# soytony/Point-Cloud-Preprocessing-Tools

Measured on AMD Instinct MI355X. Metric: BEV frames/sec (131k-pt HDL-64E cloud), higher is better.
Workload: dtype f32; 1 GPU; 1000 synthetic hdl64_sweep HDL_64E clouds per GPU (mean 135646 input pts, 133312 slots), single+multi BEV, device-resident; frames_per_gpu=1000, sub_batch=500, sensor=HDL_64E, parallelism=frames x1

## Files before the change

### point-cloud-preprocessing-tools_amd/csrc/bev_capi.hip

```cpp
#include <algorithm>
#include <cmath>
#include <cstdio>
#include <cstdlib>
#include <cstring>
#include <new>

#include <roctracer/roctx.h>

#include "bev_ctx.h"
#include "bev_libm.h"

using namespace bevk;
using namespace bevh;

namespace bevh {
void Downloader::run()
{
    (void)hipSetDevice(c->device);
    const size_t S = (size_t)c->geo.S;
    for (;;) {
        Task t;
        {
            std::unique_lock<std::mutex> lk(mu);
            cv.wait(lk, [&] { return closing || !queue.empty(); });
// ... 255 lines not shown
        HIPCK(c, hipEventRecord(c->null_ev, nullptr));
        if (!fused) HIPCK(c, hipStreamWaitEvent(c->stream, c->null_ev, 0));
        for (int q = 0; fused && q < c->n_stage_streams; ++q) HIPCK(c, hipStreamWaitEvent(c->stage_st[q], c->null_ev, 0));
    }

    int ds = 0;
    if (!identity) {
        int rc = acquire_desc(c, (size_t)n_frames, &ds);
        if (rc != BEV_OK) return rc;
        for (int f = 0; f < n_frames; ++f) {
            const uint64_t a = h_offsets[f], b = h_offsets[f + 1];
            if (b < a || b - a > c->max_points) {
                c->desc_used[ds] = false;
                return BEV_ERR_TOO_LARGE;
            }
            c->h_desc[ds][f].in_offset = a;
            c->h_desc[ds][f].n_pts = (uint32_t)(b - a);
            c->h_desc[ds][f]._pad = 0;
        }
    }

    const int sub_size = sub_frames > 0 ? std::min(sub_frames, c->max_batch) : c->max_batch;
    for (int f0 = 0; f0 < n_frames; f0 += sub_size) {
        const int nb = std::min(sub_size, n_frames - f0);
        const int q = fused ? (int)(c->sub_seq % (unsigned)c->n_stage_streams) : 0;
        hipStream_t st = fused ? c->stage_st[q] : c->stream;
        Lane &ln = c->lanes[c->sub_seq % (unsigned)c->n_lanes];
        ++c->sub_seq;
        BatchPtrs b{};
        b.pts = identity ? d_pts + (size_t)f0 * S : d_pts;
        b.frames = identity ? nullptr : ln.desc;
        b.frames_src = identity ? nullptr : c->d_desc[ds] + f0;
        b.frames_copy = identity ? nullptr : ln.desc;
        b.info = identity ? nullptr : ln.info;
        b.est = ln.est;
        b.tail_list = ln.tail_list;
        b.tail_cnt = ln.tail_cnt;
        b.cm_par = ln.cm_par;
        b.cm_sync = ln.cm_sync;
        b.winner = ln.winner;
        b.win_shift = c->win_shift;
        b.ordered = d_ordered + (size_t)f0 * S;
        b.cand = ln.cand;
        b.ncand = ln.ncand;
        b.code_main = ln.code_main;
        b.ncode = ln.ncode;
        b.ctx_tab = c->ctx_tab;
        b.avg = ln.avg;
        b.gm = d_gm ? ln.gm : nullptr;
        b.multi = d_multi ? d_multi + (size_t)f0 * c->multi_bytes : nullptr;
        b.single = d_single ? d_single + (size_t)f0 * c->single_bytes : nullptr;

        bool carried = !fused;
        auto walk = [&](int kid, int source, uint32_t mode) -> int {
            if (!carried) {
                carried = true;
                StageArgs a{};
                a.g = g;
                a.walk.b = b;
                a.walk.nf = nb;
                a.want_mode = mode;
                a.lead = c->stage_lead;
                if (!pending_is_consistent(c, q)) {
                    const int rc_ = flush_pending(c);
                    if (rc_ != BEV_OK) return rc_;
                }
                take_pending(c, &a, q);
                if (source == kSrcColMajor || source == kSrcColMajorGen) {
                    {
                        ProfScope ps(c, kid, nb, st);
                        launch_gather_ground(g, b, nb, source, mode, st);
                    }
                    a.walk.nf = 0;
                    a.lead = 0;
                    ProfScope ps(c, K_STAGE, 0, st);
                    launch_stage(a, -1, st);
                } else {
                    ProfScope ps(c, K_STAGE, nb, st);
                    launch_stage(a, source, st);
                }
                return advance_pending(c, q);
            }
            ProfScope ps(c, kid, nb, st);
            launch_gather_ground(g, b, nb, source, mode, st);
            return BEV_OK;
        };

        if (identity) {
            RoctxRange rr("bev:front (identity walk)");
            int rc = walk(K_GATHER_GROUND, kSrcIdentity, kFrameGeneral);
            if (rc != BEV_OK) return rc;
        } else {
            RoctxRange rr("bev:front (probe, column walk beside the later stages of earlier sub-batches, verdict, order scan)");
            uint32_t max_pts = 0;
            int n_exact_s = 0;
            for (int f = 0; f < nb; ++f) {
                max_pts = std::max(max_pts, c->h_desc[ds][f0 + f].n_pts);
                n_exact_s += c->h_desc[ds][f0 + f].n_pts == (uint32_t)g.S ? 1 : 0;
            }
            const uint32_t max_gen = c->win_shift <= 28 ? (1u << (32 - c->win_shift)) - 1u : 0u;
            if (ln.win_gen + 1u > max_gen) {
                HIPCK(c, hipMemsetAsync(ln.winner, 0, (size_t)c->max_batch * S * sizeof(uint32_t), st));
                ln.win_gen = 0;
            }
            if (max_gen) ++ln.win_gen;
            b.win_tag = ln.win_gen;
            {
                ProfScope ps(c, K_PROBE, nb, st);
                launch_probe(g, b, nb, c->allow_stream, c->layout_hint, st);
            }
            uint32_t seen = 0u;
            if (c->allow_stream && c->hint) {
                const uint32_t word = reinterpret_cast<volatile uint32_t *>(c->hint)[1];
                for (int m = 0; m < 8; ++m) {
                    c->mode_absent[m] = (word >> m) & 1u ? 0 : std::min(c->mode_absent[m] + 1, 1 << 20);
                    if (c->mode_absent[m] < c->mode_ttl) seen |= 1u << m;
                }
            }
            if (c->layout_hint) seen |= 1u << c->layout_hint;
            int rc = BEV_OK;
            if (c->allow_stream && ln.tail_list && (seen & (1u << kFrameStream)))
                rc = walk(K_GATHER_GROUND, kSrcInPlace, kFrameStream);
            if (rc == BEV_OK && c->allow_stream && n_exact_s > 0 && (seen & (1u << kFrameStructured)))
                rc = walk(K_WALK_STRUCTURED, kSrcStructured, kFrameStructured);
            if (rc == BEV_OK && c->allow_stream && n_exact_s > 0 && (seen & (1u << kFrameColMajor)))
                rc = walk(K_WALK_COLMAJOR, kSrcColMajor, kFrameColMajor);
            if (rc == BEV_OK && c->allow_stream && n_exact_s > 0 && ln.cm_par && (seen & (1u << kFrameColMajorGen)))
                rc = walk(K_WALK_COLMAJOR_GEN, kSrcColMajorGen, kFrameColMajorGen);
            if (rc != BEV_OK) return rc;
            if (c->allow_stream) {
                ProfScope ps(c, K_VERDICT, nb, st);
                launch_verdict(g, b, nb, c->hint, st);
            }
            {
                const bool thin = c->allow_stream && c->hint && *reinterpret_cast<volatile uint32_t *>(c->hint) == 0u;
                ProfScope ps(c, K_ORDER_SCAN, nb, st);
                launch_order_scan(g, b, nb, max_pts, thin, st);
            }
            rc = walk(K_WALK_GENERAL, kSrcGather, kFrameGeneral);
            if (rc != BEV_OK) return rc;
        }
        if (fused) {
            c->pending.push_back(bev_ctx::Pending{b, nb, d_multi != nullptr, d_single != nullptr, d_gm ? d_gm + (size_t)f0 * S : nullptr, 1, q});
        } else {
            RoctxRange rb("bev:back (cell sums, resolve, rasters)");
            {
                ProfScope ps(c, K_CELL_SUMS, nb, st);
                launch_cell_sums(g, b, nb, st);
            }
            if (d_gm) {
                ProfScope ps(c, K_GROUND_MAT, nb, st);
                launch_ground_mat(g, b, d_gm + (size_t)f0 * S, nb, st);
            }
            {
                ProfScope ps(c, K_GROUND_RESOLVE, nb, st);
                launch_ground_resolve(g, b, nb, st);
            }
            if (d_multi || d_single) {
                ProfScope ps(c, K_BEV_RASTER, nb, st);
                launch_bev_raster(g, b, d_multi != nullptr, d_single != nullptr, nb, st);
            }
        }
        c->last_sub_frames = nb;
        c->last_avg = ln.avg;
        c->last_ncode = ln.ncode;
        c->last_info = identity ? nullptr : ln.info;
        HIPCK(c, hipGetLastError());
    }
    if (fused) {
        int rc = flush ? flush_pending(c) : join_stage_streams(c);
        if (rc != BEV_OK) return rc;
    }
    if (!identity) {
        HIPCK(c, hipEventRecord(c->desc_done[ds], c->stream));
        c->desc_used[ds] = true;
    }
    return BEV_OK;
}
}

namespace {

int process_batch_host(bev_ctx_t *c, int kind, int n_frames, const void *const *in, const uint32_t *n_pts,
                       bev_point_t *const *ordered_out, uint8_t *const *multi_out, uint8_t *const *single_out,
                       int8_t *const *ground_mat_out)
{
    if (!c || n_frames < 0 || (n_frames > 0 && (!in || !n_pts || !ordered_out))) return BEV_ERR_INVALID_ARG;
    const bool raw = kind >= 0, kitti = kind == BEV_PROJECT_KITTI_HDL_64E;
    const size_t in_size = raw ? 16 : sizeof(bev_point_t);
    if (kitti && (size_t)c->geo.S > c->max_points) return BEV_ERR_TOO_LARGE;
    for (int f = 0; f < n_frames; ++f) {
        if (n_pts[f] > (kitti ? std::max(c->max_points, (size_t)c->geo.S) : c->max_points)) return BEV_ERR_TOO_LARGE;
// ... 722 lines not shown
```

### point-cloud-preprocessing-tools_amd/csrc/bev_front.h

```cpp
#ifndef BEV_FRONT_H
#define BEV_FRONT_H

#include "bev_dev.h"

namespace bevk {
using namespace bevx;

#ifndef BEV_PROBE_THREADS
#define BEV_PROBE_THREADS 256
#endif
constexpr int kProbeThreads = BEV_PROBE_THREADS;
struct ProbeLds {
    uint32_t samp[kMaxSamples];
    union {
        struct {
            uint16_t col[kCmMaxSamples], col1[kCmMaxSamples];
            uint32_t ref[kCmMaxRows], lo[kCmMaxRows], hi[kCmMaxRows], base[kCmMaxRows], misc[4];
        } cm;
        uint32_t tcnt[kTailBuckets];
    } u;
    uint32_t first_bad, overflow, struct_bad, struct_zero, cm_bad, cm_not_plain;
};
static_assert(sizeof(ProbeLds) <= kSlotLdsBytes, "a quarter of a CU's LDS");
__device__ __forceinline__ void probe_body(char *arena, const BatchPtrs &b, const Geometry &g, int allow_stream, int layout_hint, const int f)
// ... 251 lines not shown
    __syncthreads();
    uint32_t *flist = b.tail_list + (size_t)f * g.N * g.strips * kTailCap;
    auto append = [&](int row, int strip, int off, uint32_t i) {
        const int bucket = row * g.strips + strip;
        const uint32_t pos = atomicAdd(&tcnt[bucket], 1u);
        if (pos < (uint32_t)kTailCap) flist[(size_t)bucket * kTailCap + pos] = (uint32_t)off | (i << 8);
        else overflow = 1u;
    };
    constexpr int kPer = 20;
    for (uint32_t i0 = T; i0 < n; i0 += (uint32_t)kProbeThreads * kPer) {
        uint32_t rc[kPer];
#pragma unroll
        for (int k = 0; k < kPer; ++k) {
            const uint32_t i = i0 + (uint32_t)kProbeThreads * k + tid;
            rc[k] = load_once(reinterpret_cast<const uint32_t *>(fp + (i < n ? i : n - 1u)) + 5);
        }
#pragma unroll
        for (int k = 0; k < kPer; ++k) {
            const uint32_t i = i0 + (uint32_t)kProbeThreads * k + tid;
            const int row = (int)(rc[k] & 0xffffu), col = (int)(rc[k] >> 16);
            if (i >= n || row >= g.N || col >= g.H) continue;
            const int st = col / kStripCols, c = col - st * kStripCols;
            append(row, st, c + 2, i);
            if (c < 2 && st > 0) append(row, st - 1, kStripCols + 2 + c, i);
            if (c >= kStripCols - 2 && st + 1 < g.strips) append(row, st + 1, c - (kStripCols - 2), i);
            if (col >= g.H - 2 && row + 1 < g.N) append(row + 1, 0, col - (g.H - 2), i);
            if (col < 2) {
                for (int ws = g.strips - 1; ws >= 0 && ws >= g.strips - 2; --ws) {
                    const int off = g.H + col - (ws * kStripCols - 2);
                    if (off < kStripVirt && ws * kStripCols < g.H) append(row, ws, off, i);
                }
            }
        }
    }
    __syncthreads();
    PH();
    uint32_t *fcnt = b.tail_cnt + (size_t)f * g.N * g.strips;
    for (int i = tid; i < g.N * g.strips; i += kProbeThreads) {
        const int r = i / g.strips, st = i - r * g.strips;
        fcnt[st * g.N + r] = tcnt[i] < (uint32_t)kTailCap ? tcnt[i] : (uint32_t)kTailCap;
    }
    if (tid == 0) b.info[f] = overflow ? FrameInfo{0u, kFrameGeneral, 4u, 0u} : FrameInfo{T, kFrameStream, 0u, 0u};
    PH();
    TL_END(K_PROBE);
    PH_PRINT("probe samples prefix-end estimates tail-lists counts", tid == 0 && f == 100);
}
__global__ __launch_bounds__(kProbeThreads) void k_probe(BatchPtrs b, Geometry g, int allow_stream, int layout_hint)
{
    __shared__ __attribute__((aligned(16))) char arena[sizeof(ProbeLds)];
    probe_body(arena, b, g, allow_stream, layout_hint, (int)blockIdx.x);
}


__global__ __launch_bounds__(1024) void k_verdict(FrameInfo *info, int nf, uint32_t *host_hint, const uint32_t *cm_sync, int N)
{
    __shared__ uint32_t others, modes;
    if (threadIdx.x == 0) others = modes = 0u;
    __syncthreads();
    uint32_t mine = 0u, mask = 0u;
    for (int f = threadIdx.x; f < nf; f += 1024) {
        FrameInfo fi = info[f];
        mask |= 1u << (fi.mode & 31u);
        bool bad_stream = ((fi.mode == kFrameStream || fi.mode == kFrameColMajor) && (fi.failed != 0u || fi.consumed != fi.T)) ||
                          (fi.mode == kFrameColMajorGen && ((fi.failed & kInfoFailed) != 0u || fi.consumed != fi.T));
        if (fi.mode == kFrameColMajorGen && !bad_stream && (fi.failed & (kInfoCmUsed | kInfoCmStray)) != 0u && cm_sync) {
            const uint32_t *win0 = cm_sync + (size_t)f * kCmSyncWords + kCmPubWords, *used0 = win0 + kCmMaxRows, *stray = used0 + kCmMaxRows;
            for (int r = 0; r < N && r < kCmMaxRows; ++r) {
                const uint32_t u = used0[r];
                if ((u & kCmUsedBit) != 0u && (u & ~kCmUsedBit) != win0[r]) bad_stream = true;
                if (stray[r] > win0[r]) bad_stream = true;
            }
        }
        const bool bad_struct = fi.mode == kFrameStructured &&
                                ((fi.failed & kInfoFailed) != 0u || fi.consumed != fi.T ||
                                 ((fi.failed & kInfoZeroSeen) != 0u) != ((fi.failed & kInfoZeroGuess) != 0u));
        if (bad_stream || bad_struct) {
            info[f].mode = kFrameRedo;
            fi.mode = kFrameRedo;
        }
        mine += frame_read_in_place(fi.mode) ? 0u : 1u;
    }
    if (mine) atomicAdd(&others, mine);
    if (mask) atomicOr(&modes, mask);
    __syncthreads();
    if (threadIdx.x == 0 && host_hint) {
        __hip_atomic_store(host_hint, others, __ATOMIC_RELAXED, __HIP_MEMORY_SCOPE_SYSTEM);
        __hip_atomic_store(host_hint + 1, modes, __ATOMIC_RELAXED, __HIP_MEMORY_SCOPE_SYSTEM);
    }
}

constexpr int kSeenBits = 11;
constexpr int kScanPerThread = 4;
constexpr int kScanIdxBits = 10;
constexpr int kScanRowBins = 128;
__global__ __launch_bounds__(256) void k_order_scan(const bev_point_t *__restrict__ pts,
                                                    const FrameDesc *__restrict__ frames,
                                                    const FrameInfo *__restrict__ info,
                                                    uint32_t *__restrict__ winner, int N, int H, int S,
                                                    uint32_t tag_bits)
{
    const int f = blockIdx.y;
    if (info && frame_read_in_place(info[f].mode)) return;
    const FrameDesc fd = frames[f];
    const bev_point_t *fp = pts + fd.in_offset;
    uint32_t *fw = winner + (size_t)f * S;
    __shared__ uint32_t any_spread2[2];
    __shared__ uint32_t row_fill[kScanRowBins];
    __shared__ uint32_t pairs[256 * kScanPerThread];
    static_assert(256 * kScanPerThread == (1 << kScanIdxBits), "bits of block-local index");
  uint32_t turn = 0u;
  for (uint32_t blk = blockIdx.x; blk * (256u * kScanPerThread) < fd.n_pts; blk += gridDim.x, ++turn) {
    uint32_t &any_spread = any_spread2[turn & 1u];
    const uint32_t block0 = blk * (256u * kScanPerThread);
    const uint32_t base = block0 + threadIdx.x;
    uint32_t slot[kScanPerThread];
    bool spread = false;
    uint32_t rcw[kScanPerThread];
#pragma unroll
    for (int k = 0; k < kScanPerThread; ++k) {
        const uint32_t i = base + 256u * k;
        rcw[k] = load_once(reinterpret_cast<const uint32_t *>(fp + (i < fd.n_pts ? i : fd.n_pts - 1u)) + 5);
    }
#pragma unroll
    for (int k = 0; k < kScanPerThread; ++k) {
        const uint32_t i = base + 256u * k;
        const uint32_t row = rcw[k] & 0xffffu, col = rcw[k] >> 16;
        slot[k] = (i < fd.n_pts && row < (uint32_t)N && col < (uint32_t)H) ? row * (uint32_t)H + col
                                                                                         : 0xffffffffu;
    }
#pragma unroll
    for (int k = 0; k < kScanPerThread; ++k) {
        const unsigned long long vm = __ballot(slot[k] != 0xffffffffu);
        if (vm) {
            const int lo_lane = __ffsll((long long)vm) - 1, hi_lane = 63 - __clzll((long long)vm);
            const uint32_t a = __shfl(slot[k], lo_lane), z = __shfl(slot[k], hi_lane);
            const uint32_t d = a > z ? a - z : z - a;
            spread = spread || d > 4u * (uint32_t)H;
        }
    }
    if (threadIdx.x == 0) any_spread = 0u;
    __syncthreads();
    if (spread && (threadIdx.x & 63) == 0) any_spread = 1u;
    __syncthreads();
    if (any_spread == 0u || N > kScanRowBins || S > (1 << (32 - kScanIdxBits))) {
#pragma unroll
        for (int k = 0; k < kScanPerThread; ++k)
            if (slot[k] != 0xffffffffu) atomicMax(&fw[slot[k]], tag_bits | (base + 256u * k + 1u));
        continue;
    }
    for (int r = threadIdx.x; r < kScanRowBins; r += 256) row_fill[r] = 0u;
#pragma unroll
    for (int k = 0; k < kScanPerThread; ++k) pairs[threadIdx.x + 256u * k] = 0xffffffffu;
    __syncthreads();
    uint32_t rank[kScanPerThread];
#pragma unroll
    for (int k = 0; k < kScanPerThread; ++k)
        rank[k] = slot[k] != 0xffffffffu ? atomicAdd(&row_fill[slot[k] / (uint32_t)H], 1u) : 0u;
    __syncthreads();
    if (threadIdx.x < 64) {
        const uint32_t c0 = row_fill[2 * threadIdx.x], c1 = row_fill[2 * threadIdx.x + 1];
        uint32_t incl = c0 + c1;
#pragma unroll
        for (int d = 1; d < 64; d <<= 1) {
            const uint32_t v = __shfl_up(incl, d);
            if ((int)threadIdx.x >= d) incl += v;
        }
        row_fill[2 * threadIdx.x] = incl - c0 - c1;
        row_fill[2 * threadIdx.x + 1] = incl - c1;
    }
    __syncthreads();
#pragma unroll
    for (int k = 0; k < kScanPerThread; ++k)
        if (slot[k] != 0xffffffffu)
            pairs[row_fill[slot[k] / (uint32_t)H] + rank[k]] = (slot[k] << kScanIdxBits) | (threadIdx.x + 256u * k);
    __syncthreads();
#pragma unroll
    for (int k = 0; k < kScanPerThread; ++k) {
        const uint32_t j = threadIdx.x + 256u * k;
        const uint32_t pr = pairs[j];
        if (pr != 0xffffffffu) atomicMax(&fw[pr >> kScanIdxBits], tag_bits | (block0 + (pr & ((1u << kScanIdxBits) - 1u)) + 1u));
    }
  }
}

}

#endif
```

### point-cloud-preprocessing-tools_amd/csrc/bev_internal.h

```cpp
#ifndef BEV_INTERNAL_H
#define BEV_INTERNAL_H

#include <hip/hip_runtime.h>
#include <stdint.h>

#include "../../include/bev_mi355x.h"
#include "bev_exact.h"

namespace bevk {

constexpr int kGatherThreads = 256;
constexpr int kSlotsPerThread = 4;
constexpr int kTile = kGatherThreads * kSlotsPerThread;
constexpr int kMaxTiles = 1024;
constexpr int kStripThreads = 256;
constexpr int kStripCols = 236;
constexpr int kStripVirt = kStripCols + 4;
constexpr int kSeg = 256;
constexpr int kMaxSegs = 1024;
constexpr int kSumWaves = 4;
constexpr int kSumThreads = kSumWaves * 64;
constexpr int kStageThreads = 256;
constexpr int kSlotLdsBytes = 32 * 1280;
constexpr int kResolveThreads = kStageThreads;
constexpr int kResolveParts = 4;
#ifndef BEV_RESOLVE_WGS
#define BEV_RESOLVE_WGS 2
#endif
constexpr int kResolveWgs = BEV_RESOLVE_WGS;
static_assert(kResolveParts % kResolveWgs == 0, "whole parts per workgroup");
constexpr int kRasterThreads = kStageThreads;
constexpr int kRasterLdsCap = kSlotLdsBytes;
constexpr int kRasterFineDiv = bevx::kBandFineDiv;
constexpr int kRasterSplit = 8;
constexpr int kMaxBands = bevx::kBandMax;
constexpr int kMaxStrips = 280;
constexpr int kCodeListCap = 4096;
constexpr int kCtxTabWords = bevx::kGridRows + bevx::kGridCols + 512 / 4;

struct FrameDesc {
    uint64_t in_offset;
    uint32_t n_pts;
    uint32_t _pad;
};

enum : uint32_t { kFrameGeneral = 0, kFrameStream = 1, kFrameRedo = 2, kFrameStructured = 3, kFrameColMajor = 4, kFrameColMajorGen = 5 };
__host__ __device__ inline bool frame_read_in_place(uint32_t mode) { return mode == kFrameStream || mode == kFrameStructured || mode == kFrameColMajor || mode == kFrameColMajorGen; }
struct FrameInfo {
    uint32_t T;
    uint32_t mode;
    uint32_t consumed;
    uint32_t failed;
};
constexpr uint32_t kInfoFailed = 1u, kInfoZeroSeen = 2u, kInfoZeroGuess = 4u;
constexpr uint32_t kInfoCmStray = 8u;
constexpr uint32_t kInfoCmUsed = 16u;
constexpr int kProbeStride = 63, kProbeStrideDense = 127;
constexpr int kMaxSamples = 4096;
constexpr int kStreamMinPrefix = 2048;
constexpr int kTailCap = 64;
constexpr int kTailMax = 16384;
constexpr int kTailBuckets = 2048;
constexpr int kPlainDisp = 8;
constexpr int kColMaxDisp = 12;
constexpr int kCmSpread = 18;
constexpr int kCmProbeDisp = kColMaxDisp;
constexpr int kCmExt = 16;
constexpr int kCmMaxRows = 128;
constexpr int kCmMaxSamples = 4096;
constexpr int kCmParWords = 4 + kCmMaxRows;
constexpr uint32_t kCmUsedBit = 0x80000000u;
constexpr int kCmMaxStrips = 16;
constexpr int kCmPubWords = (kCmMaxRows / 2) * kCmMaxStrips * 2;
constexpr int kCmSyncWords = kCmPubWords + 3 * kCmMaxRows;
constexpr int kStreamMaxRows = 64;

static_assert(sizeof(bev_point_t) == 32, "bev_point_t must be 32 bytes");

struct Geometry {
    int N, H, G;
    int S;
    int tiles;
    int strips;
    int segs;
    int raster_bands;
    int emitters;
    uint32_t code_cap;
    uint32_t code_stride;
    bevx::RasterParams rp;
};
// ... 44 lines not shown
    K_WALK_COLMAJOR_GEN,
    K_VERDICT,
    K_STAGE,
    K_RF_CELLS,
    K_RF_TOP,
    K_RF_VOXEL,
    K_RF_NORMALS,
    K_ICP_GRID,
    K_ICP,
    K_ICP_BEST,
    K_FINE_VOXEL,
    K_FINE_GRID,
    K_FINE_ICP,
    K_KITTI_CROSSINGS,
    K_KITTI_CHAIN,
    K_KITTI_ASSIGN,
    K_KITTI_GATHER,
    K_FLOAT_BEV_BATCH,
    K_POSED_SPLAT,
    K_POSED_EXPAND,
    K_SUBMAP_SPLAT,
    K_SUBMAP_FLOAT_SPLAT,
    K_SUBMAP_TARGET,
    K_SUBMAP_ICP,
    K_SUBMAP_VOX_MOVE,
    K_SUBMAP_VOX_KEYS,
    K_SUBMAP_VOX_TILE,
    K_SUBMAP_VOX_GLOBAL,
    K_SUBMAP_VOX_FINISH,
    K_SUBMAP_VOX_OUT,
    K_SUBMAP_PN_TARGET,
    K_SUBMAP_COARSE_ICP,
    K_COUNT
};
const char *kernel_name(int id);
int raster_bands_for(int mat_size);

struct StagePart {
    BatchPtrs b;
    int nf;
};
struct StageArgs {
    Geometry g;
    StagePart walk, sums, resolve, raster;
    uint32_t want_mode;
    int want_multi, want_single;
    int lead;
};
void launch_stage(const StageArgs &a, int source, hipStream_t st);
size_t stage_lds_bytes(const Geometry &g, int source);

void launch_order_scan(const Geometry &g, const BatchPtrs &b, int nf, uint32_t max_pts, bool thin, hipStream_t st);
enum : int { kSrcGather = 0, kSrcIdentity = 1, kSrcInPlace = 2, kSrcStructured = 3, kSrcColMajor = 4, kSrcColMajorGen = 5 };
void launch_gather_ground(const Geometry &g, const BatchPtrs &b, int nf, int source, uint32_t mode, hipStream_t st);
void launch_probe(const Geometry &g, const BatchPtrs &b, int nf, bool allow_stream, int layout_hint , hipStream_t st);
void launch_verdict(const Geometry &g, const BatchPtrs &b, int nf, uint32_t *host_hint, hipStream_t st);
void launch_gather_only(const Geometry &g, const BatchPtrs &b, int nf, hipStream_t st);
void launch_cell_sums(const Geometry &g, const BatchPtrs &b, int nf, hipStream_t st);
void launch_ground_resolve(const Geometry &g, const BatchPtrs &b, int nf, hipStream_t st);
void launch_bev_raster(const Geometry &g, const BatchPtrs &b, bool want_multi, bool want_single, int nf, hipStream_t st);
void launch_bev_raster_dense(const Geometry &g, const uint32_t *codes, uint32_t n_codes, uint8_t *multi, uint8_t *single,
                             hipStream_t st);
void launch_ground_mat(const Geometry &g, const BatchPtrs &b, int8_t *out, int nf, hipStream_t st);
void launch_cloud_codes(const Geometry &g, const bev_point_t *cloud, uint32_t n, uint32_t *codes, hipStream_t st);
void launch_float_bev(const bev_point_t *cloud, uint32_t n, float interval, int M, bool skip_label0, float *grid,
                      hipStream_t st);
void launch_transform(const bev_point_t *cloud, uint32_t n, const float m[12], bev_point_t *out, hipStream_t st);
struct ProjFrame {
    uint64_t off;
    uint32_t n;
    uint32_t blk0;
};
constexpr int kProjPerThread = 4;
constexpr int kProjBlock = 256 * kProjPerThread;
void launch_project_batch(int kind, const float *xyzi, const ProjFrame *tab, int nf, uint32_t blocks, bev_point_t *out,
                          hipStream_t st);
constexpr int kKittiGroup = BEV_PROJECT_KITTI_GROUP;
struct KittiHeader {
    int32_t ring0;
    uint32_t n_links;
    uint32_t link[68];
};
struct KittiWork {
    KittiHeader *hdr;
    int32_t *col;
    uint32_t *cnt;
    uint32_t *pos;
    uint32_t *winner;
    uint32_t n_cap, blocks_cap;
};
void launch_project_kitti(int step, const float *xyzi, const ProjFrame *tab, int nf, uint32_t n_max, const KittiWork &w,
                          bev_point_t *out, hipStream_t st);
void launch_float_bev_batch(const bev_point_t *clouds, const ProjFrame *tab, int nf, uint32_t blocks, const float *poses,
                            int n_poses, float interval, int M, bool skip_label0, float *grids, hipStream_t st);
void launch_posed_splat(const bev_point_t *clouds, const ProjFrame *tab, int nf, uint32_t blocks, const float *poses, int n_poses,
                        const Geometry &g, uint32_t *planes, hipStream_t st);
void launch_posed_expand(const Geometry &g, const uint32_t *planes, int n_grids, uint8_t *multi, uint8_t *single, hipStream_t st);
void launch_submap_splat(const bev_point_t *clouds, const void *rows, const uint32_t *ent0, int nf, uint32_t blocks,
                         const void *entries, const Geometry &g, uint32_t *planes, hipStream_t st);
void launch_submap_float_splat(const bev_point_t *clouds, const void *rows, const uint32_t *ent0, int nf, uint32_t blocks,
                               const void *entries, float interval, int M, bool skip_label0, float *grids, hipStream_t st);
void launch_angle_debug(const float *dx, const float *dy, const float *dz, uint8_t *out, size_t n, hipStream_t st);
constexpr int kRfThreads = 256;
constexpr int kRfGrid = 10;
constexpr int kRfCells = kRfGrid * kRfGrid;
constexpr int kRfMinCellPoints = 20;
constexpr int kRfLdsKeys = 8192;
// ... 147 lines not shown
```

### point-cloud-preprocessing-tools_amd/csrc/bev_kernels.hip

```cpp
#include <algorithm>
#include <cstdlib>
#include <type_traits>

#include "bev_internal.h"
#include "bev_libm.h"

#include "bev_dev.h"
#include "bev_front.h"
#include "bev_walk.h"
#include "bev_cell_sums.h"
#include "bev_resolve.h"
#include "bev_raster.h"
#include "bev_misc.h"
#include "bev_project.h"
#include "bev_manip.h"
#include "bev_posed.h"
#include "bev_submap.h"
#include "bev_submap_float.h"
#include "bev_reg_common.h"
#include "bev_regfront.h"
#include "bev_icp.h"
#include "bev_fine.h"
#include "bev_submap_reg.h"
#include "bev_submap_vox.h"
// ... 68 lines not shown
    else if (!gm) fn(std::false_type{}, std::false_type{});
    else fn(std::false_type{}, std::true_type{});
}
static bool raster_is_pow2(const Geometry &g) { return g.rp.inv_interval != 0.0f && g.rp.inv_height_res != 0.0f; }
constexpr int stage_source(int src) { return (src == kSrcColMajor || src == kSrcColMajorGen) ? (int)kSrcGather : src; }

size_t stage_lds_bytes(const Geometry &g, int source)
{
    const size_t w = with_source(source, [](auto s) { return sizeof(WalkLds<stage_source(decltype(s)::value)>); });
    const size_t others = std::max(std::max(SumDims::lds_bytes(g.segs), sizeof(ResolveLds)), raster_lds_bytes(g));
    return std::max(w, others);
}
void launch_stage(const StageArgs &a, int source, hipStream_t st)
{
    if (a.walk.nf == 0) source = kSrcInPlace;
    const Geometry &g = a.g;
    const bool gm = a.walk.nf > 0 && a.walk.b.gm != nullptr;
    const int back = std::max(a.sums.nf, std::max(a.resolve.nf, a.raster.nf));
    const int lead = back > 0 ? a.lead : 0;
    const int slots = std::max((a.walk.nf + 7) / 8, back > 0 ? (back + 7) / 8 + lead : 0);
    if (slots == 0) return;
    const int per_slot = g.strips + kSumQ + kResolveWgs + g.raster_bands;
    const dim3 gr((unsigned)(8 * slots * per_slot)), bl(kStageThreads);
    const size_t lds = stage_lds_bytes(g, source);
    StageArgs args = a;
    args.lead = lead;
    with_source(source, [&](auto s) {
        constexpr int kSrc = stage_source(decltype(s)::value);
        with_variant(raster_is_pow2(g), gm, [&](auto p, auto m) {
            hipLaunchKernelGGL((k_stage<kSrc, decltype(p)::value, decltype(m)::value>), gr, bl, lds, st, args);
        });
    });
}

hipError_t configure_kernels(const Geometry &g)
{
    hipError_t e = hipFuncSetAttribute(reinterpret_cast<const void *>(k_cell_sums),
                                       hipFuncAttributeMaxDynamicSharedMemorySize, (int)SumDims::lds_bytes(kMaxSegs));
    if (e != hipSuccess) return e;
    e = hipFuncSetAttribute(reinterpret_cast<const void *>(k_bev_raster), hipFuncAttributeMaxDynamicSharedMemorySize,
                            (int)raster_lds_bytes(g));
    if (e != hipSuccess) return e;
    e = hipFuncSetAttribute(reinterpret_cast<const void *>(k_posed_expand), hipFuncAttributeMaxDynamicSharedMemorySize,
                            (int)raster_lds_bytes(g));
    if (e != hipSuccess) return e;
    return hipFuncSetAttribute(reinterpret_cast<const void *>(k_bev_raster_dense),
                               hipFuncAttributeMaxDynamicSharedMemorySize, (int)raster_lds_bytes(g));
}
void launch_order_scan(const Geometry &g, const BatchPtrs &b, int nf, uint32_t max_pts, bool thin, hipStream_t st)
{
    if (max_pts == 0 || nf == 0) return;
    const unsigned per_block = 256u * kScanPerThread;
    const unsigned blocks = (max_pts + per_block - 1u) / per_block;
    dim3 grid(thin && blocks > 8u ? 8u : blocks, (unsigned)nf);
    hipLaunchKernelGGL(k_order_scan, grid, dim3(256), 0, st, b.pts, b.frames, b.info, b.winner, g.N, g.H, g.S,
                       b.win_tag << b.win_shift);
}
void launch_gather_ground(const Geometry &g, const BatchPtrs &b, int nf, int source, uint32_t mode, hipStream_t st)
{
    if (nf == 0) return;
    const dim3 gr(xcd_grid(nf, g.strips)), bl(kStripThreads);
    with_source(source, [&](auto s) {
        constexpr int kSrc = decltype(s)::value;
        with_variant(raster_is_pow2(g), b.gm != nullptr, [&](auto p, auto m) {
            hipLaunchKernelGGL((k_walk<kSrc, decltype(p)::value, decltype(m)::value>), gr, bl, 0, st, b, g, nf, mode);
        });
    });
}
void launch_probe(const Geometry &g, const BatchPtrs &b, int nf, bool allow_stream, int layout_hint, hipStream_t st)
{
    if (nf == 0) return;
    hipLaunchKernelGGL(k_probe, dim3(nf), dim3(kProbeThreads), 0, st, b, g, allow_stream ? 1 : 0, layout_hint);
}
void launch_verdict(const Geometry &g, const BatchPtrs &b, int nf, uint32_t *host_hint, hipStream_t st)
{
    if (nf == 0) return;
    hipLaunchKernelGGL(k_verdict, dim3(1), dim3(1024), 0, st, b.info, nf, host_hint, b.cm_sync, g.N);
}
void launch_gather_only(const Geometry &g, const BatchPtrs &b, int nf, hipStream_t st)
{
    if (nf == 0) return;
    hipLaunchKernelGGL(k_gather_only, dim3(xcd_grid(nf, g.tiles)), dim3(kGatherThreads), 0, st, b, g, nf);
}
void launch_cell_sums(const Geometry &g, const BatchPtrs &b, int nf, hipStream_t st)
{
    if (nf == 0) return;
    hipLaunchKernelGGL(k_cell_sums, dim3(xcd_grid(nf, kSumQ)), dim3(kSumThreads), SumDims::lds_bytes(g.segs), st, b, g, nf);
}
void launch_ground_resolve(const Geometry &g, const BatchPtrs &b, int nf, hipStream_t st)
{
    if (nf == 0) return;
    const bool pow2 = g.rp.inv_interval != 0.0f && g.rp.inv_height_res != 0.0f;
    if (pow2) hipLaunchKernelGGL(k_ground_resolve<true>, dim3(nf * kResolveWgs), dim3(kResolveThreads), 0, st, b, g);
    else hipLaunchKernelGGL(k_ground_resolve<false>, dim3(nf * kResolveWgs), dim3(kResolveThreads), 0, st, b, g);
}
void launch_bev_raster(const Geometry &g, const BatchPtrs &b, bool want_multi, bool want_single, int nf, hipStream_t st)
{
    if (nf == 0) return;
    hipLaunchKernelGGL(k_bev_raster, dim3(8 * ((nf + 7) / 8) * g.raster_bands), dim3(kRasterThreads), raster_lds_bytes(g), st, b,
                       g, nf, want_multi ? 1 : 0, want_single ? 1 : 0);
}
void launch_bev_raster_dense(const Geometry &g, const uint32_t *codes, uint32_t n_codes, uint8_t *multi, uint8_t *single,
                             hipStream_t st)
{
    hipLaunchKernelGGL(k_bev_raster_dense, dim3(g.raster_bands), dim3(kRasterThreads), raster_lds_bytes(g), st, codes,
                       n_codes, multi, single, g.rp);
}
void launch_ground_mat(const Geometry &g, const BatchPtrs &b, int8_t *out, int nf, hipStream_t st)
{
    if (nf == 0) return;
    hipLaunchKernelGGL(k_ground_mat, dim3(xcd_grid(nf, g.tiles)), dim3(kGatherThreads), 0, st, b, g, out, nf);
}
void launch_cloud_codes(const Geometry &g, const bev_point_t *cloud, uint32_t n, uint32_t *codes, hipStream_t st)
{
    if (n == 0) return;
    hipLaunchKernelGGL(k_cloud_codes, dim3((n + 255u) / 256u), dim3(256), 0, st, cloud, n, codes, g.rp);
}
void launch_float_bev(const bev_point_t *cloud, uint32_t n, float interval, int M, bool skip_label0, float *grid,
                      hipStream_t st)
{
    if (n == 0) return;
    hipLaunchKernelGGL(k_float_bev, dim3((n + 255u) / 256u), dim3(256), 0, st, cloud, n, interval, M,
                       skip_label0 ? 1 : 0, reinterpret_cast<uint32_t *>(grid));
}
void launch_transform(const bev_point_t *cloud, uint32_t n, const float m[12], bev_point_t *out, hipStream_t st)
{
    if (n == 0) return;
    Affine34 a;
    for (int k = 0; k < 12; ++k) a.m[k] = m[k];
    hipLaunchKernelGGL(k_transform, dim3((n + 255u) / 256u), dim3(256), 0, st, cloud, n, a, out);
// ... 65 lines not shown
```

### point-cloud-preprocessing-tools_amd/csrc/bev_walk.h

```cpp
#ifndef BEV_WALK_H
#define BEV_WALK_H

#include "bev_dev.h"

#ifndef BEV_SEENB
#define BEV_SEENB 8
#endif

namespace bevk {
using namespace bevx;

struct WalkRow {
    u32x4 lo, hi;
    uint32_t code, key, fl;
};
__device__ __forceinline__ int wr_status(uint32_t fl) { return (int)(fl & 3u) - 1; }
__device__ __forceinline__ int wr_gflag(uint32_t fl) { return (int)((fl >> 2) & 3u) - 1; }

__device__ __forceinline__ uint32_t quarter_scan(bool c, uint32_t q, uint32_t *rank)
{
    const uint32_t sh = q << 3;
    const uint32_t one = c ? 1u << sh : 0u;
    uint32_t x = one;
    x += (uint32_t)__builtin_amdgcn_update_dpp(0, (int)x, 0x111 , 0xf, 0xf, false);
// ... 25 lines not shown
    const int own_cols;
    const int row_span;
    const bool last_strip;
    const char *const fbytes;
    const uint32_t T;
    const uint32_t ring_l;
    __device__ __forceinline__ WalkCol(const Geometry &g, int strip_, const void *points, uint32_t T_, uint32_t ring_l_)
        : N(g.N), H(g.H), strip(strip_), strips(g.strips), tid((int)threadIdx.x), lane(tid & 63), wv(__builtin_amdgcn_readfirstlane(tid >> 6)),
          v(strip_ * kStripCols + tid - 2), vcol(v >= H ? v - H : v), provider(tid < kStripVirt && (v < H + 2) && (v >= 0 || strip_ == 0)),
          outcol(tid >= 2 && tid < 2 + kStripCols && v < H), first_col(strip_ * kStripCols - 2),
          own_cols((H - first_col - 2) < kStripCols ? (H - first_col - 2) : kStripCols), row_span((H - first_col) < kStripVirt ? (H - first_col) : kStripVirt),
          last_strip(strip_ * kStripCols - 2 + kStripVirt > H), fbytes(reinterpret_cast<const char *>(points)), T(T_), ring_l(ring_l_)
    {
    }
};

template <int kSrc>
struct WalkSource;
#ifdef BEV_CS_CLOCK
#define WALK_PHA_PARAMS , long long (&pha_)[8], long long &pha_t
#define WALK_PHA_ARGS , pha_, pha_t
#else
#define WALK_PHA_PARAMS
#define WALK_PHA_ARGS
#endif

template <int kSrc>
struct WalkLds {
    static constexpr int kWaves = kStripThreads / 64;
    static constexpr int kSeenB = WalkSource<kSrc>::kIndexed ? BEV_SEENB : kSeenBits;
    alignas(16) char ring[WalkSource<kSrc>::kRingBytes];
    alignas(16) u32x4 zero16[1];
    alignas(16) float4 edge[3][kWaves][4];
    alignas(16) uint32_t wave_cnt[2][2 * kWaves];
    uint32_t band_cursor[kMaxBands];
    uint32_t seen[1 << kSeenB];
    int edge_x[kGridRows], edge_y[kGridCols];
    uint8_t band_tab[512];
    typename WalkSource<kSrc>::Lds src;
};

}

#include "bev_walk_gather.h"
#include "bev_walk_inplace.h"
#include "bev_walk_firing.h"

namespace bevk {

static_assert(sizeof(WalkLds<kSrcInPlace>) <= 32 * 1280 && sizeof(WalkLds<kSrcGather>) <= 32 * 1280 && sizeof(WalkLds<kSrcStructured>) <= 32 * 1280,
              "four column-walk workgroups per CU: 32 of the CU's 128 LDS granules (1,280 bytes) each");
static_assert(sizeof(WalkLds<kSrcColMajorGen>) <= 42 * 1280 && sizeof(WalkLds<kSrcColMajor>) <= 42 * 1280, "three firing-order workgroups per CU");

template <int kSrc, bool kPow2, bool kGm>
__device__ __forceinline__ void walk_body(char *arena, const BatchPtrs &b, const Geometry &g, const int f, int strip, uint32_t want_mode, int bid )
{
    TL_BEGIN;
    using Source = WalkSource<kSrc>;
    using Lds = WalkLds<kSrc>;
    constexpr bool kIndexed = Source::kIndexed;
#ifdef BEV_CS_CLOCK
    const long long tl_t0 = wall_clock64();
#endif
    (void)bid;
    if (Source::kStrip0Last) strip = g.strips - 1 - strip;
    if (!Source::kAnyMode && b.info) {
        const uint32_t fmode = b.info[f].mode;
        if (frame_read_in_place(want_mode) ? fmode != want_mode : frame_read_in_place(fmode)) return;
    }
    constexpr int kWaves = Lds::kWaves, kSeenB = Lds::kSeenB;
    Lds &lds_w = *reinterpret_cast<Lds *>(arena);
    const WalkCol c(g, strip, Source::input(b, g, f), kIndexed ? b.info[f].T : 0u, __builtin_amdgcn_readfirstlane(lds_addr(&lds_w.ring[0])));
    const int tid = c.tid, lane = c.lane, wv = c.wv, v = c.v;
    const bool outcol = c.outcol;
    const int N = g.N, H = g.H, lo_row = g.N - g.G, strips = g.strips;
    const size_t frame_off = (size_t)f * g.S;
    const int bands = g.raster_bands;

    const int sh_right = ((lane + 2) & 63) << 2, sh_left = ((lane - 2) & 63) << 2;
    auto from_right2 = [&](float x) -> float { return __uint_as_float((uint32_t)__builtin_amdgcn_ds_bpermute(sh_right, (int)__float_as_uint(x))); };
    auto from_left2 = [&](float x) -> float { return __uint_as_float((uint32_t)__builtin_amdgcn_ds_bpermute(sh_left, (int)__float_as_uint(x))); };

    auto &ring = lds_w.ring;
    auto &edge = lds_w.edge;
    auto &wave_cnt = lds_w.wave_cnt;
    auto &band_cursor = lds_w.band_cursor;
    auto &band_tab = lds_w.band_tab;
    auto &seen = lds_w.seen;
    auto &edge_x = lds_w.edge_x;
    auto &edge_y = lds_w.edge_y;
    Source src(lds_w, c, b, g, f);
    if (tid < kMaxBands) band_cursor[tid] = 0u;
    if (tid < 4 * kWaves) (&wave_cnt[0][0])[tid] = 0u;
    if (tid < 3 * kWaves * 4) (&edge[0][0][0])[tid] = make_float4(0.f, 0.f, 0.f, 0.f);
    for (int k = tid; k < (1 << kSeenB); k += kStripThreads) seen[k] = kSkip;
    for (int x = tid; x < g.rp.mat_size; x += kStripThreads) band_tab[x] = (uint8_t)raster_band_of_nodiv(x, g.rp);
    if (tid < kGridRows) edge_x[tid] = cell_edge_bin(tid, 75.0f, g.rp);
    else if (tid < kGridRows + kGridCols) edge_y[tid - kGridRows] = cell_edge_bin(tid - kGridRows, 50.0f, g.rp);
    src.setup();
    lds_barrier();
    if (!kIndexed && __ballot(c.provider) == 0ull) return;

    src.prologue();

    WalkRow pr[3] = {};
    PHA_DECL;
#ifdef BEV_CS_CLOCK
    if (lane == 0 && bid == 100) printf("walk_prologue %lld (x10 ns)\n", pha_t - tl_t0);
#endif
    float zref = __uint_as_float(0x7fc00000u);

    const size_t cand_base = (size_t)f * g.segs * kSeg;
    const gptr<u32x2> fcand = (gptr<u32x2>)(b.cand + cand_base);
    const gptr<uint32_t> fncand = (gptr<uint32_t>)(b.ncand + (size_t)f * g.segs);
    const uint32_t code_last = in_vgpr(g.code_cap - 1u), code_stride = in_vgpr(g.code_stride);
    const gptr<uint32_t> flist = (gptr<uint32_t>)(b.code_main + ((size_t)f * g.emitters + strip) * bands * (size_t)g.code_stride);
    const gptr<u32x4> fordered = (gptr<u32x4>)(b.ordered + frame_off);
    const gptr<int8_t> fgm = (gptr<int8_t>)(kGm ? b.gm + frame_off : nullptr);
    RasterParams rp = g.rp;
    rp.max_range_f = in_vgpr(rp.max_range_f);
    rp.lidar_to_ground = in_vgpr(rp.lidar_to_ground);
    rp.mat_size = in_vgpr(rp.mat_size);
    rp.n_layers = in_vgpr(rp.n_layers);
    if (kPow2) {
        rp.inv_interval = in_vgpr(rp.inv_interval);
        rp.inv_height_res = in_vgpr(rp.inv_height_res);
    } else {
        rp.interval = in_vgpr(rp.interval);
        rp.height_res = in_vgpr(rp.height_res);
    }
    const uint32_t xp_sw = ((uint32_t)lane >> 2) & 1u;
    const uint32_t xp_w = (uint32_t)wv * 1024u + (uint32_t)(lane & 31) * 32u + (lane < 32 ? 0u : 4096u);
    const uint32_t xp_wlo = xp_w + 16u * xp_sw, xp_whi = xp_w + 16u * (xp_sw ^ 1u);
    const uint32_t xp_unit = ((uint32_t)lane & ~1u) | (((uint32_t)lane & 1u) ^ (((uint32_t)lane >> 3) & 1u));
    const uint32_t xp_r0 = (uint32_t)wv * 1024u + xp_unit * 16u, xp_r1 = xp_r0 + 4096u;

    uint32_t ord_off = (uint32_t)((-2 * H + strip * kStripCols - 2 + 64 * wv) * 2 + 64 + lane) * 16u;
    const uint32_t row_bytes = (uint32_t)H * 32u;
    auto row_step = [&](auto I, const int r) {
        constexpr int kI = decltype(I)::value;
        WalkRow &p0 = pr[RingSlots<kI>::s0], &p1 = pr[RingSlots<kI>::s2], &p2 = pr[RingSlots<kI>::s1];
        const int par = r & 1;
        u32x4 cur_lo, cur_hi;
        PHA(7);
        src.template arrive<kI>(r, cur_lo, cur_hi WALK_PHA_ARGS);
        if constexpr (!kIndexed) {
            if (lane < 2 || lane >= 62)
                edge[r % 3][wv][lane < 2 ? lane : lane - 60] = make_float4(__uint_as_float(cur_lo.x), __uint_as_float(cur_lo.y), __uint_as_float(cur_lo.z), __uint_as_float(cur_hi.x));
            const bool c2 = outcol && wr_gflag(p2.fl) == 1;
            const uint32_t q2 = p2.key & 3u;
            uint32_t rank2;
            const uint32_t scan = quarter_scan(c2, q2, &rank2);
            if (lane == 63) wave_cnt[par][kWaves + wv] = scan;
            p2.fl |= rank2 << kFlRankShift;
// ... 118 lines not shown

        if constexpr (kIndexed) {
            if (lane < 2 || lane >= 62) edge[r % 3][wv][lane < 2 ? lane : lane - 60] = make_float4(cur.x, cur.y, cur.z, cur.i);
            const uint32_t q1 = p1.key & 3u;
            uint32_t rank1;
            const uint32_t scan = quarter_scan(cand1, q1, &rank1);
            if (lane == 63) wave_cnt[par ^ 1][kWaves + wv] = scan;
            p1.fl |= rank1 << kFlRankShift;
        }
    };
    for (int r0 = 0; r0 < N + 2; r0 += 3) {
        row_step(std::integral_constant<int, 0>{}, r0);
        if (r0 + 1 < N + 2) row_step(std::integral_constant<int, 1>{}, r0 + 1);
        if (r0 + 2 < N + 2) row_step(std::integral_constant<int, 2>{}, r0 + 2);
    }
    wait_vm<0>();
#ifdef BEV_CS_CLOCK
    src.clk_print(bid, f WALK_PHA_ARGS);
    if (tid == 0 && kIndexed && bid < kWalkTlCap) {
        long long *rec = g_walk_tl[bid];
        rec[0] = tl_t0;
        rec[1] = wall_clock64();
        rec[2] = (long long)(unsigned)__builtin_amdgcn_s_getreg((31 << 11) | 4);
        rec[3] = (long long)(unsigned)__builtin_amdgcn_s_getreg((31 << 11) | 20);
    }
#endif
    lds_barrier();
    if (tid < bands) b.ncode[((size_t)f * g.emitters + strip) * bands + tid] = band_cursor[tid];
    src.finish();
    if constexpr (Source::kChecked) {
        uint32_t consumed = src.consumed, failed = src.failed;
#pragma unroll
        for (int d = 32; d >= 1; d >>= 1) {
            consumed += __shfl_xor(consumed, d);
            failed |= __shfl_xor(failed, d);
        }
        if (lane == 0) {
            atomicAdd(&b.info[f].consumed, consumed);
            if (failed) atomicOr(&b.info[f].failed, failed);
        }
    }
    TL_END(K_GATHER_GROUND);
}

template <int kSrc, bool kPow2, bool kGm>
__global__ __launch_bounds__(kStripThreads, (kSrc == kSrcColMajor || kSrc == kSrcColMajorGen) ? 3 : 4) void k_walk(BatchPtrs b, Geometry g, int nf, uint32_t want_mode)
{
    __shared__ __attribute__((aligned(16))) char arena[sizeof(WalkLds<kSrc>)];
    int f, strip;
    if (!map_block_xcd((int)blockIdx.x, nf, g.strips, f, strip)) return;
    walk_body<kSrc, kPow2, kGm>(arena, b, g, f, strip, want_mode, (int)blockIdx.x);
}

}

#endif
```

Measured before the change: 427,900 frames/s.

## Launch tiny persistent order-scan and walk grids when verdict says no frames need redo

When the host hint shows no frame fell back to the general path, the order scan and general walk now launch a small persistent grid of a few workers. Each worker first checks whether any of its frames need work and exits early if none do, and otherwise loops over frames and strips itself. Before this, those launches used full-size grids that mostly exited right away. The verdict kernel also drops from 1024 to 256 threads. This cuts launch and block-scheduling overhead in the common all-in-place case. The cost is that any frames that do need the general path are processed serially by very few workgroups.

```diff
diff --git a/point-cloud-preprocessing-tools_amd/csrc/bev_capi.hip b/point-cloud-preprocessing-tools_amd/csrc/bev_capi.hip
--- a/point-cloud-preprocessing-tools_amd/csrc/bev_capi.hip
+++ b/point-cloud-preprocessing-tools_amd/csrc/bev_capi.hip
@@ -331,7 +331,7 @@
         b.single = d_single ? d_single + (size_t)f0 * c->single_bytes : nullptr;
 
         bool carried = !fused;
-        auto walk = [&](int kid, int source, uint32_t mode) -> int {
+        auto walk = [&](int kid, int source, uint32_t mode, bool thin = false) -> int {
             if (!carried) {
                 carried = true;
                 StageArgs a{};
@@ -348,7 +348,7 @@
                 if (source == kSrcColMajor || source == kSrcColMajorGen) {
                     {
                         ProfScope ps(c, kid, nb, st);
-                        launch_gather_ground(g, b, nb, source, mode, st);
+                        launch_gather_ground(g, b, nb, source, mode, false, st);
                     }
                     a.walk.nf = 0;
                     a.lead = 0;
@@ -361,7 +361,7 @@
                 return advance_pending(c, q);
             }
             ProfScope ps(c, kid, nb, st);
-            launch_gather_ground(g, b, nb, source, mode, st);
+            launch_gather_ground(g, b, nb, source, mode, thin, st);
             return BEV_OK;
         };
 
@@ -411,12 +411,12 @@
                 ProfScope ps(c, K_VERDICT, nb, st);
                 launch_verdict(g, b, nb, c->hint, st);
             }
+            const bool thin = c->allow_stream && c->hint && *reinterpret_cast<volatile uint32_t *>(c->hint) == 0u;
             {
-                const bool thin = c->allow_stream && c->hint && *reinterpret_cast<volatile uint32_t *>(c->hint) == 0u;
                 ProfScope ps(c, K_ORDER_SCAN, nb, st);
                 launch_order_scan(g, b, nb, max_pts, thin, st);
             }
-            rc = walk(K_WALK_GENERAL, kSrcGather, kFrameGeneral);
+            rc = walk(K_WALK_GENERAL, kSrcGather, kFrameGeneral, thin);
             if (rc != BEV_OK) return rc;
         }
         if (fused) {
diff --git a/point-cloud-preprocessing-tools_amd/csrc/bev_front.h b/point-cloud-preprocessing-tools_amd/csrc/bev_front.h
--- a/point-cloud-preprocessing-tools_amd/csrc/bev_front.h
+++ b/point-cloud-preprocessing-tools_amd/csrc/bev_front.h
@@ -327,13 +327,14 @@
 }
 
 
-__global__ __launch_bounds__(1024) void k_verdict(FrameInfo *info, int nf, uint32_t *host_hint, const uint32_t *cm_sync, int N)
+constexpr int kVerdictThreads = 256;
+__global__ __launch_bounds__(kVerdictThreads) void k_verdict(FrameInfo *info, int nf, uint32_t *host_hint, const uint32_t *cm_sync, int N)
 {
     __shared__ uint32_t others, modes;
     if (threadIdx.x == 0) others = modes = 0u;
     __syncthreads();
     uint32_t mine = 0u, mask = 0u;
-    for (int f = threadIdx.x; f < nf; f += 1024) {
+    for (int f = threadIdx.x; f < nf; f += kVerdictThreads) {
         FrameInfo fi = info[f];
         mask |= 1u << (fi.mode & 31u);
         bool bad_stream = ((fi.mode == kFrameStream || fi.mode == kFrameColMajor) && (fi.failed != 0u || fi.consumed != fi.T)) ||
@@ -371,19 +372,25 @@
 __global__ __launch_bounds__(256) void k_order_scan(const bev_point_t *__restrict__ pts,
                                                     const FrameDesc *__restrict__ frames,
                                                     const FrameInfo *__restrict__ info,
-                                                    uint32_t *__restrict__ winner, int N, int H, int S,
+                                                    uint32_t *__restrict__ winner, int nf, int N, int H, int S,
                                                     uint32_t tag_bits)
 {
-    const int f = blockIdx.y;
-    if (info && frame_read_in_place(info[f].mode)) return;
-    const FrameDesc fd = frames[f];
-    const bev_point_t *fp = pts + fd.in_offset;
-    uint32_t *fw = winner + (size_t)f * S;
     __shared__ uint32_t any_spread2[2];
     __shared__ uint32_t row_fill[kScanRowBins];
     __shared__ uint32_t pairs[256 * kScanPerThread];
     static_assert(256 * kScanPerThread == (1 << kScanIdxBits), "bits of block-local index");
+  if (info && gridDim.y < (unsigned)nf) {
+    int any = 0;
+    for (int f = (int)blockIdx.y + (int)gridDim.y * (int)threadIdx.x; f < nf; f += (int)gridDim.y * 256)
+        any |= frame_read_in_place(info[f].mode) ? 0 : 1;
+    if (!__syncthreads_or(any)) return;
+  }
   uint32_t turn = 0u;
+  for (int f = blockIdx.y; f < nf; f += gridDim.y) {
+    if (info && frame_read_in_place(info[f].mode)) continue;
+    const FrameDesc fd = frames[f];
+    const bev_point_t *fp = pts + fd.in_offset;
+    uint32_t *fw = winner + (size_t)f * S;
   for (uint32_t blk = blockIdx.x; blk * (256u * kScanPerThread) < fd.n_pts; blk += gridDim.x, ++turn) {
     uint32_t &any_spread = any_spread2[turn & 1u];
     const uint32_t block0 = blk * (256u * kScanPerThread);
@@ -456,6 +463,7 @@
         if (pr != 0xffffffffu) atomicMax(&fw[pr >> kScanIdxBits], tag_bits | (block0 + (pr & ((1u << kScanIdxBits) - 1u)) + 1u));
     }
   }
+  }
 }
 
 }
diff --git a/point-cloud-preprocessing-tools_amd/csrc/bev_internal.h b/point-cloud-preprocessing-tools_amd/csrc/bev_internal.h
--- a/point-cloud-preprocessing-tools_amd/csrc/bev_internal.h
+++ b/point-cloud-preprocessing-tools_amd/csrc/bev_internal.h
@@ -36,6 +36,11 @@
 constexpr int kMaxBands = bevx::kBandMax;
 constexpr int kMaxStrips = 280;
 constexpr int kCodeListCap = 4096;
+#ifndef BEV_REDO_WORKERS
+#define BEV_REDO_WORKERS 8
+#endif
+constexpr int kRedoWorkers = BEV_REDO_WORKERS;
+static_assert(kRedoWorkers >= 1, "someone has to look");
 constexpr int kCtxTabWords = bevx::kGridRows + bevx::kGridCols + 512 / 4;
 
 struct FrameDesc {
@@ -186,7 +191,7 @@
 
 void launch_order_scan(const Geometry &g, const BatchPtrs &b, int nf, uint32_t max_pts, bool thin, hipStream_t st);
 enum : int { kSrcGather = 0, kSrcIdentity = 1, kSrcInPlace = 2, kSrcStructured = 3, kSrcColMajor = 4, kSrcColMajorGen = 5 };
-void launch_gather_ground(const Geometry &g, const BatchPtrs &b, int nf, int source, uint32_t mode, hipStream_t st);
+void launch_gather_ground(const Geometry &g, const BatchPtrs &b, int nf, int source, uint32_t mode, bool thin, hipStream_t st);
 void launch_probe(const Geometry &g, const BatchPtrs &b, int nf, bool allow_stream, int layout_hint , hipStream_t st);
 void launch_verdict(const Geometry &g, const BatchPtrs &b, int nf, uint32_t *host_hint, hipStream_t st);
 void launch_gather_only(const Geometry &g, const BatchPtrs &b, int nf, hipStream_t st);
diff --git a/point-cloud-preprocessing-tools_amd/csrc/bev_kernels.hip b/point-cloud-preprocessing-tools_amd/csrc/bev_kernels.hip
--- a/point-cloud-preprocessing-tools_amd/csrc/bev_kernels.hip
+++ b/point-cloud-preprocessing-tools_amd/csrc/bev_kernels.hip
@@ -144,13 +144,19 @@
     if (max_pts == 0 || nf == 0) return;
     const unsigned per_block = 256u * kScanPerThread;
     const unsigned blocks = (max_pts + per_block - 1u) / per_block;
-    dim3 grid(thin && blocks > 8u ? 8u : blocks, (unsigned)nf);
-    hipLaunchKernelGGL(k_order_scan, grid, dim3(256), 0, st, b.pts, b.frames, b.info, b.winner, g.N, g.H, g.S,
+    const dim3 grid(thin ? 1u : blocks, thin ? (unsigned)std::min(nf, kRedoWorkers) : (unsigned)nf);
+    hipLaunchKernelGGL(k_order_scan, grid, dim3(256), 0, st, b.pts, b.frames, b.info, b.winner, nf, g.N, g.H, g.S,
                        b.win_tag << b.win_shift);
 }
-void launch_gather_ground(const Geometry &g, const BatchPtrs &b, int nf, int source, uint32_t mode, hipStream_t st)
-{
-    if (nf == 0) return;
+void launch_gather_ground(const Geometry &g, const BatchPtrs &b, int nf, int source, uint32_t mode, bool thin, hipStream_t st)
+{
+    if (nf == 0) return;
+    if (thin && source == kSrcGather && b.info) {
+        with_variant(raster_is_pow2(g), b.gm != nullptr, [&](auto p, auto m) {
+            hipLaunchKernelGGL((k_walk_thin<decltype(p)::value, decltype(m)::value>), dim3((unsigned)std::min(nf, kRedoWorkers)), dim3(kStripThreads), 0, st, b, g, nf);
+        });
+        return;
+    }
     const dim3 gr(xcd_grid(nf, g.strips)), bl(kStripThreads);
     with_source(source, [&](auto s) {
         constexpr int kSrc = decltype(s)::value;
@@ -167,7 +173,7 @@
 void launch_verdict(const Geometry &g, const BatchPtrs &b, int nf, uint32_t *host_hint, hipStream_t st)
 {
     if (nf == 0) return;
-    hipLaunchKernelGGL(k_verdict, dim3(1), dim3(1024), 0, st, b.info, nf, host_hint, b.cm_sync, g.N);
+    hipLaunchKernelGGL(k_verdict, dim3(1), dim3(kVerdictThreads), 0, st, b.info, nf, host_hint, b.cm_sync, g.N);
 }
 void launch_gather_only(const Geometry &g, const BatchPtrs &b, int nf, hipStream_t st)
 {
diff --git a/point-cloud-preprocessing-tools_amd/csrc/bev_walk.h b/point-cloud-preprocessing-tools_amd/csrc/bev_walk.h
--- a/point-cloud-preprocessing-tools_amd/csrc/bev_walk.h
+++ b/point-cloud-preprocessing-tools_amd/csrc/bev_walk.h
@@ -101,7 +101,7 @@
               "four column-walk workgroups per CU: 32 of the CU's 128 LDS granules (1,280 bytes) each");
 static_assert(sizeof(WalkLds<kSrcColMajorGen>) <= 42 * 1280 && sizeof(WalkLds<kSrcColMajor>) <= 42 * 1280, "three firing-order workgroups per CU");
 
-template <int kSrc, bool kPow2, bool kGm>
+template <int kSrc, bool kPow2, bool kGm, bool kLoop = false>
 __device__ __forceinline__ void walk_body(char *arena, const BatchPtrs &b, const Geometry &g, const int f, int strip, uint32_t want_mode, int bid )
 {
     TL_BEGIN;
@@ -148,7 +148,7 @@
     else if (tid < kGridRows + kGridCols) edge_y[tid - kGridRows] = cell_edge_bin(tid - kGridRows, 50.0f, g.rp);
     src.setup();
     lds_barrier();
-    if (!kIndexed && __ballot(c.provider) == 0ull) return;
+    if (!kIndexed && !kLoop && __ballot(c.provider) == 0ull) return;
 
     src.prologue();
 
@@ -373,6 +373,25 @@
     walk_body<kSrc, kPow2, kGm>(arena, b, g, f, strip, want_mode, (int)blockIdx.x);
 }
 
-}
-
-#endif
+template <bool kPow2, bool kGm>
+__global__ __launch_bounds__(kStripThreads, 4) void k_walk_thin(BatchPtrs b, Geometry g, int nf)
+{
+    __shared__ __attribute__((aligned(16))) char arena[sizeof(WalkLds<kSrcGather>)];
+    {
+        int any = 0;
+        for (int f = (int)blockIdx.x + (int)gridDim.x * (int)threadIdx.x; f < nf; f += (int)gridDim.x * kStripThreads)
+            any |= frame_read_in_place(b.info[f].mode) ? 0 : 1;
+        if (!__syncthreads_or(any)) return;
+    }
+    for (int f = (int)blockIdx.x; f < nf; f += (int)gridDim.x) {
+        if (frame_read_in_place(b.info[f].mode)) continue;
+        for (int strip = 0; strip < g.strips; ++strip) {
+            walk_body<kSrcGather, kPow2, kGm, true>(arena, b, g, f, strip, kFrameGeneral, (int)blockIdx.x);
+            lds_barrier();
+        }
+    }
+}
+
+}
+
+#endif
```

Result: slower. 418,200 frames/s (-2.3%).
